# LanceZPF/loongx

Measured on AMD Instinct MI355X. Metric: edited images/s @512x512, 28-step Flux denoise, higher is better.
Workload: dtype bf16

## Files before the change

### loongx_amd/csrc/gemm.hip

```cpp
#include "gemm8.h"


static double round_us(int bm, int K) { return bm == 256 ? 15.0 + 1.81 * (K / 64) : 10.5 + 1.06 * (K / 64); }

struct GemmEnv { int bm, g4, sk, g4_fault; };
static int env_int(const char* name, int dflt) {
  const char* s = getenv(name);
  return s ? atoi(s) : dflt;
}
static GemmEnv read_gemm_env() { return GemmEnv{env_int("LX_GEMM_BM", 0), env_int("LX_GEMM4", 1), env_int("LX_GEMM4_SK", 1), env_int("LX_GEMM4_FAULT", 0)}; }
static GemmEnv g_gemm_env = read_gemm_env();
static const GemmEnv& gemm_env() { return g_gemm_env; }
extern "C" void lx_gemm_reload_env(void) { g_gemm_env = read_gemm_env(); }

namespace {
constexpr size_t SK_FLAGS_OFF = (size_t)256 * SK_SLOT_FLOATS * sizeof(float);
constexpr size_t SK_WS_BYTES = SK_FLAGS_OFF + (256 + 64) * sizeof(int);
static_assert(SK_WS_BYTES % 256 == 0, "workspace size keeps the 256-byte alignment contract");
constexpr int SK_MIN_KT_ALL = 96;
constexpr int SK_MAX_ROUNDS = 16;

int device_cus() {
  static int n = -1;
  if (n < 0) {
    int dev = 0;
    hipDeviceProp_t pr;
    n = (hipGetDevice(&dev) == hipSuccess && hipGetDeviceProperties(&pr, dev) == hipSuccess) ? pr.multiProcessorCount : 0;
  }
  return n;
}
}

static long tiles_of(const lx_gemm_desc& p, int bm) { return (long)((p.M + bm - 1) / bm) * ((p.N + BN - 1) / BN); }

static lx_gemm_desc sub_rows(const lx_gemm_desc& p, int r0, int rows) {
  lx_gemm_desc q = p;
  q.A = (const uint16_t*)p.A + (size_t)r0 * p.lda;
  const int epi = p.epilogue & 0xff;
  q.C = epi == LX_EPI_STORE_BF16 ? (void*)((uint16_t*)p.C + (size_t)r0 * p.ldc) : (void*)((float*)p.C + (size_t)r0 * p.ldc);
  if (p.lora_t) q.lora_t = p.lora_t + (size_t)r0 * p.lora_ldt;
  if (p.qkv_k) q.qkv_k = (uint16_t*)p.qkv_k + (size_t)r0 * p.qkv_k_ld;
  if (p.qkv_q8) {
    q.qkv_q8 = (uint8_t*)p.qkv_q8 + (size_t)r0 * p.qkv_ld8;
// ... 1 lines not shown
  }
  q.M = rows;
  return q;
}

static int launch_plan(const GemmArgs& a, int bm, hipStream_t s, int variant = LX_GV_BF16) {
  if (a.n == 0) return LX_OK;
  if (variant == LX_GV_SPLIT) lx_gemm8_launch_split(bm, a, s);
  else if (variant == LX_GV_F16) lx_gemm8_launch_f16(bm, a, s);
  else if (variant == LX_GV_FP8) lx_gemm8_launch_fp8(bm, a, s);
  else lx_gemm8_launch_bf16(bm, a, s);
  LX_LAUNCH_CHECK("lx_gemm_bf16");
  return LX_OK;
}

void lx_gemm8_launch_bf16(int bm, const GemmArgs& a, hipStream_t s) {
  const int t = a.tile_start[a.n];
  if (bm == 256) hipLaunchKernelGGL((lx_gemm_kernel<256, false>), dim3(t), dim3(NTHREADS), 0, s, a);
  else hipLaunchKernelGGL((lx_gemm_kernel<128, false>), dim3(t), dim3(NTHREADS), 0, s, a);
}
void lx_gemm8_mixed_launch_bf16(const GemmArgs& big, const GemmArgs& tail, int n_big_pad, hipStream_t s) {
  hipLaunchKernelGGL(lx_gemm_mixed_kernel<false>, dim3(n_big_pad + tail.tile_start[tail.n]), dim3(NTHREADS), 0, s, big, tail, n_big_pad);
}

static void plan_add(GemmArgs& a, const lx_gemm_desc& p, int m_base, int bm) {
  a.p[a.n] = p;
  a.m_base[a.n] = m_base;
  a.tile_start[a.n + 1] = a.tile_start[a.n] + (int)tiles_of(p, bm);
  ++a.n;
  for (int i = a.n + 1; i <= MAX_SUB; ++i) a.tile_start[i] = a.tile_start[a.n];
}

static thread_local int lx_gemm_last = LX_GEMM_PLAN_NONE;
extern "C" int lx_gemm_last_plan(void) { return lx_gemm_last; }
static int planned(int rc, int plan) {
  if (rc == LX_OK) lx_gemm_last = plan;
  return rc;
}

extern "C" size_t lx_gemm_workspace_bytes(void) { return SK_WS_BYTES; }

extern "C" int lx_gemm_workspace_status(void* workspace, void* stream) {
  LX_CHECK_ARG(workspace, "lx_gemm_workspace_status: NULL workspace");
  int* err = (int*)((char*)workspace + SK_FLAGS_OFF) + 256;
  int v = 0;
  hipStream_t s = (hipStream_t)stream;
  if (hipMemcpyAsync(&v, err, sizeof(int), hipMemcpyDeviceToHost, s) != hipSuccess || hipStreamSynchronize(s) != hipSuccess) {
    lx_set_error("lx_gemm_workspace_status: reading the error word failed: %s", hipGetErrorString(hipGetLastError()));
    return LX_ERR_LAUNCH;
  }
  if (v == 0) return LX_OK;
  (void)hipMemsetAsync((char*)workspace + SK_FLAGS_OFF, 0, (256 + 64) * sizeof(int), s);
  (void)hipStreamSynchronize(s);
  lx_set_error("lx_gemm_bf16_ws: a split-K pair workgroup timed out waiting for its partner (CUs held by other work?); the results "
               "of that launch are invalid. Re-run with the workspace omitted (lx_gemm_bf16) or LX_GEMM4_SK=0");
  return LX_ERR_LAUNCH;
}

extern "C" int lx_gemm_bf16(const lx_gemm_desc* problems, int n, void* stream) { return lx_gemm_bf16_ws(problems, n, nullptr, 0, stream); }

extern "C" int lx_gemm_bf16_ws(const lx_gemm_desc* problems, int n, void* workspace, size_t ws_bytes, void* stream) {
  LX_CHECK_ARG(problems && n >= 1 && n <= LX_GEMM_MAX_GROUP, "lx_gemm_bf16: n=%d out of range [1,%d]", n, LX_GEMM_MAX_GROUP);
  long t256 = 0, t128 = 0;
  int kmax = 0;
  bool split = false, fp8 = false, f16 = false, qkv = false;
  for (int i = 0; i < n; ++i) fp8 = fp8 || (problems[i].epilogue & LX_OPERANDS_FP8) != 0;
  for (int i = 0; i < n; ++i) f16 = f16 || (problems[i].epilogue & LX_OPERANDS_F16) != 0;
  for (int i = 0; i < n; ++i) {
    const lx_gemm_desc& p = problems[i];
// ... 91 lines not shown
    bool split_all = can_split && full == 0 && kt_all >= SK_MIN_KT_ALL;
    const int tail_div = !qkv && kt_all >= 96 ? 2 : 3;
    bool split_tail = can_split && full > 0 && tail * tail_div <= NCU;
    int np = 2;
    if (!split && env.sk != 2 && kt_all >= 24 && tail * 3 <= 256 && tail * 3 <= NCU && (split_all || split_tail) && (kt_all >= 96 || tail * 6 <= NCU)) np = 3;
    if (split) {
      const double r4 = 8.9 + 1.31 * kt_all;
      const bool sk_tail = can_split && tail > 0;
      const double c4 = (double)(full / NCU) * r4 + (tail == 0 ? 0.0 : sk_tail ? 8.9 + 1.31 * (kt_all - kt_all / 2) + 6.0 : r4);
      const double c8a = (double)((t256 + NCU - 1) / NCU) * (5.8 + 1.55 * kt_all), c8b = (double)((t128 + NCU - 1) / NCU) * (10.5 + 1.06 * kt_all);
      fills = env.g4 == 2 || c4 < (c8a < c8b ? c8a : c8b);
      split_all = fills && sk_tail && full == 0;
      split_tail = fills && sk_tail && full > 0;
      if (!fills) split_all = split_tail = false;
    }
    if (ok && (fills || split_all || split_tail)) {
      GemmArgs all;
      all.n = 0;
      all.tile_start[0] = 0;
      for (int i = 1; i <= MAX_SUB; ++i) all.tile_start[i] = 0;
      for (int i = 0; i < n; ++i) plan_add(all, problems[i], 0, 256);
      float* slots = nullptr;
      int *flags = nullptr, *err = nullptr;
      unsigned grid = (unsigned)t256;
      int sk_full = (int)t256, sk_parts = 1;
      if (split_all || split_tail) {
        slots = (float*)workspace;
        flags = (int*)((char*)workspace + SK_FLAGS_OFF);
        err = flags + 256;
        grid = (unsigned)(full + np * tail);
        sk_full = (int)full;
        sk_parts = env.g4_fault ? 3 : 2;
      }
      if (split) lx_gemm4_launch_split(all, grid, sk_full, sk_parts, slots, flags, err, s);
      else if (f16) lx_gemm4_launch_f16(all, grid, sk_full, sk_parts, slots, flags, err, s, np);
      else lx_gemm4_launch_bf16(all, grid, sk_full, sk_parts, slots, flags, err, s, np);
      LX_LAUNCH_CHECK("lx_gemm_bf16");
      return planned(LX_OK, !(split_all || split_tail) ? LX_GEMM_PLAN_G4 : np == 3 ? LX_GEMM_PLAN_G4_SPLIT3 : LX_GEMM_PLAN_G4_SPLIT2);
    }
  }
  if (split) {
    const double ca = (double)((t256 + NCU - 1) / NCU) * round_us(256, kmax), cb = (double)((t128 + NCU - 1) / NCU) * round_us(128, kmax);
    const int bm = forced ? forced : (cb < ca ? 128 : 256);
    GemmArgs all;
    all.n = 0;
    all.tile_start[0] = 0;
    for (int i = 1; i <= MAX_SUB; ++i) all.tile_start[i] = 0;
    for (int i = 0; i < n; ++i) plan_add(all, problems[i], 0, bm);
    return planned(launch_plan(all, bm, s, LX_GV_SPLIT), bm == 256 ? LX_GEMM_PLAN_8WAVE_256 : LX_GEMM_PLAN_8WAVE_128);
  }
  if (workspace) LX_CHECK_ARG(ws_bytes >= SK_WS_BYTES && ((uintptr_t)workspace & 255) == 0, "lx_gemm_bf16_ws: workspace needs %zu bytes (lx_gemm_workspace_bytes()), 256-byte aligned", SK_WS_BYTES);
  const int variant = f16 ? LX_GV_F16 : LX_GV_BF16;
  const double c_a = (double)((t256 + NCU - 1) / NCU) * round_us(256, kmax);
  const double c_b = (double)((t128 + NCU - 1) / NCU) * round_us(128, kmax);
  GemmArgs big, tail;
  big.n = tail.n = 0;
  big.tile_start[0] = tail.tile_start[0] = 0;
  for (int i = 1; i <= MAX_SUB; ++i) big.tile_start[i] = tail.tile_start[i] = 0;
  double c_c = 1e30;
  const long full = (t256 / NCU) * NCU;
  if (forced == 0 && full > 0 && t256 > full) {
    long remain = t256;
    int keep_rows[LX_GEMM_MAX_GROUP];
    for (int i = 0; i < n; ++i) keep_rows[i] = problems[i].M;
    for (int i = n - 1; i >= 0 && remain > full; --i) {
      const int tn = (problems[i].N + BN - 1) / BN;
      while (remain > full && keep_rows[i] > 0) {
        const int last_rows = keep_rows[i] % 256 ? keep_rows[i] % 256 : 256;
        keep_rows[i] -= last_rows;
        remain -= tn;
      }
// ... 34 lines not shown
```

### loongx_amd/csrc/gemm4.h

```cpp
#pragma once
#include "gemm_common.h"

namespace {

constexpr int G4_STAGE = 256 * BK * 2 + BN * BK * 2;
constexpr int G4_LDS = 2 * G4_STAGE;
constexpr int G4_PLD = 132;
constexpr int G4_PATCHES = 4 * 2 * 16 * G4_PLD * 4;
constexpr int G4_SLOT = 8 * 1024;
constexpr int G4_SMEM = G4_PATCHES + 4 * 2 * G4_SLOT > G4_LDS ? G4_PATCHES + 4 * 2 * G4_SLOT : G4_LDS;
static_assert(G4_LDS <= G4_SMEM && G4_SMEM <= 160 * 1024 && G4_PATCHES % 1024 == 0 && G4_PATCHES + 4 * 2 * G4_SLOT <= G4_SMEM,
              "LDS budget / epilogue patches / row ring");

#ifdef LX_G4_PROBE
__device__ unsigned long long lx_g4_probe_buf[8192 * 8];
#define G4_STAMP(k) if (threadIdx.x == 0 && blockIdx.x < 8192) { asm volatile("s_waitcnt lgkmcnt(0)" ::: "memory"); lx_g4_probe_buf[blockIdx.x * 8 + (k)] = __builtin_amdgcn_s_memtime(); }
#else
#define G4_STAMP(k)
#endif


template <bool SPLIT, bool F16 = false, int NP = 2>
__global__ __launch_bounds__(G4_THREADS) void lx_gemm4_kernel(const GemmArgs args, const int sk_full, const int sk_parts, float* __restrict__ sk_slots,
                                                              int* __restrict__ sk_flags, int* __restrict__ sk_err) {
#if defined(__HIP_DEVICE_COMPILE__)
  __shared__ __attribute__((aligned(1024))) char smem[G4_SMEM];
  constexpr int BM = 256, A_BYTES = BM * BK * 2;
  const int pid = blockIdx.x;
  G4_STAMP(0)
  const int total = args.tile_start[MAX_SUB];
  int lid, part = 0;
  if (pid < sk_full) {
    const int q = sk_full >> 3, r = sk_full & 7;
    const int xcd = pid & 7, inx = pid >> 3;
    lid = (xcd < r ? xcd * (q + 1) : r * (q + 1) + (xcd - r) * q) + inx;
  } else {
    const int r = pid - sk_full;
    lid = sk_full + r / NP;
    part = r % NP;
  }
  (void)total;
  const bool split_tile = pid >= sk_full && sk_parts >= 2;
  const int g = tile_group(args, lid);
  lx_gemm_desc P = args.p[g];
  int tm, tn;
  tile_coords<BM>(P, lid - args.tile_start[g], tm, tn);
  const int tid = threadIdx.x, lane = tid & 63;
  const int wave = __builtin_amdgcn_readfirstlane(tid >> 6);
  const int wm = wave >> 1, wn = wave & 1, l15 = lane & 15, lq = lane >> 4;
  int m0 = tm * BM, n0 = tn * BN;
  int M = P.M, N = P.N;
  const int K = P.K;
  const bool w_tiled = (P.epilogue & LX_W_TILED) != 0;
  const int nk1 = K / BK;
  const int nkt = SPLIT ? nk1 * max(P.k_segs, 1) : nk1;
// ... 188 lines not shown
    __syncthreads();
    __builtin_amdgcn_fence(__ATOMIC_RELEASE, "workgroup");
    if (tid == 0) {
      const int me = pid - sk_full, other = NP == 2 ? (me ^ 1) : (me - part + (part + 1) % NP), other2 = me - part + (part + 2) % NP;
      bool ok = __hip_atomic_load(sk_err, __ATOMIC_RELAXED, __HIP_MEMORY_SCOPE_AGENT) == 0;
      if (ok) {
        if (!(sk_parts == 3 && part == 1))
          __hip_atomic_store(sk_flags + me, NP - 1, __ATOMIC_RELAXED, __HIP_MEMORY_SCOPE_AGENT);
        int spins = 0;
        while (__hip_atomic_load(sk_flags + other, __ATOMIC_RELAXED, __HIP_MEMORY_SCOPE_AGENT) == 0) {
          __builtin_amdgcn_s_sleep(1);
          if (++spins > (1 << 20)) { ok = false; break; }
        }
        if constexpr (NP == 3) {
          while (ok && __hip_atomic_load(sk_flags + other2, __ATOMIC_RELAXED, __HIP_MEMORY_SCOPE_AGENT) == 0) {
            __builtin_amdgcn_s_sleep(1);
            if (++spins > (1 << 20)) { ok = false; break; }
          }
        }
        if (ok) {
          if constexpr (NP == 2) __hip_atomic_store(sk_flags + other, 0, __ATOMIC_RELAXED, __HIP_MEMORY_SCOPE_AGENT);
          else {
            __hip_atomic_fetch_add(sk_flags + other, -1, __ATOMIC_RELAXED, __HIP_MEMORY_SCOPE_AGENT);
            __hip_atomic_fetch_add(sk_flags + other2, -1, __ATOMIC_RELAXED, __HIP_MEMORY_SCOPE_AGENT);
          }
        } else __hip_atomic_store(sk_err, 1, __ATOMIC_RELAXED, __HIP_MEMORY_SCOPE_AGENT);
      }
    }
    __syncthreads();
    G4_STAMP(6)
    __builtin_amdgcn_fence(__ATOMIC_ACQUIRE, "workgroup");
  };

  const int epi = P.epilogue & 0xff;
  const bool do_gelu = (P.epilogue & LX_EPI_GELU) != 0;
  const int mw0 = m0 + wm * 128, nw0 = n0 + wn * 128;
  float* patch = (float*)smem + wave * (2 * 16 * G4_PLD);
  const bool bf16_out = epi == LX_EPI_STORE_BF16;
  const int c8 = (lane & 15) * 8, c4 = (lane & 31) * 4;
  const int ncol = nw0 + (bf16_out ? c8 : c4);
  const bool col_ok = ncol < N;
  f32x4 bias0 = {0.f, 0.f, 0.f, 0.f}, bias1 = {0.f, 0.f, 0.f, 0.f};
  if (P.bias && col_ok) {
    bias0 = *(const f32x4*)(P.bias + ncol);
    if (bf16_out) bias1 = *(const f32x4*)(P.bias + ncol + 4);
  }
  asm volatile("s_waitcnt vmcnt(0)" : "+v"(bias0), "+v"(bias1)::"memory");
  const bool gelu0 = do_gelu && ncol >= P.gelu_col_start;
  const int m_base = args.m_base[g];
  static_assert(!(F16 && SPLIT), "fp16 operands exclude the split-bf16 mode");
  float f16_mx = 0.f;
  const bool qkv_tile = (P.epilogue & LX_EPI_QKV) != 0 && n0 < 3 * P.qkv_d;
  const int qkind = qkv_tile ? n0 / P.qkv_d : -1;
  f32x4 nw0v = {1.f, 1.f, 1.f, 1.f}, nw1v = {1.f, 1.f, 1.f, 1.f};
  if (qkv_tile && qkind != 1) {
    const float* nwp = (qkind == 2 ? P.qkv_norm_q : P.qkv_norm_k) + c8;
    nw0v = *(const f32x4*)nwp; nw1v = *(const f32x4*)(nwp + 4);
    asm volatile("s_waitcnt vmcnt(0)" : "+v"(nw0v), "+v"(nw1v)::"memory");
  }
#ifdef LX_G4_RESID_GLOBAL
  constexpr bool RING_RES = false;
#else
  constexpr bool RING_RES = true;
#endif
#ifdef LX_G4_ROPE_GLOBAL
  constexpr bool RING_ROPE = false;
#else
  constexpr bool RING_ROPE = true;
#endif
  char* const ring = smem + G4_PATCHES + wave * (2 * G4_SLOT);
  const bool ring_res = RING_RES && epi == LX_EPI_RESID_F32 && !qkv_tile;
  const bool ring_rope = RING_ROPE && qkv_tile && qkind != 1;
  const int ring_lane = ring_rope ? ((lane >> 4) * 128 + c8) * 4 : min(ncol, max(N - 4, 0)) * 4;
  const int ring_mlast = M - 1 - mw0;
  auto ring_issue = [&](int b, int s) {
    const lx_rsrc_t rs_row = lx_make_rsrc(ring_rope ? (const void*)P.qkv_rope : (const void*)((const float*)P.C + (size_t)min(mw0, M - 1) * P.ldc));
    if (ring_rope) {
      const int gm = m_base + mw0 + b * 16, p0 = gm - (gm / P.rows_per_batch) * P.rows_per_batch;
#pragma unroll
      for (int p_ = 0; p_ < 8; ++p_)
        lx_buf_to_lds(rs_row, (lptr_t)(ring + s * G4_SLOT + p_ * 1024), (uint32_t)ring_lane, (p0 + (p_ >> 1) * 4) * 512 + (p_ & 1) * 16);
    } else {
#pragma unroll
      for (int t = 0; t < 8; ++t) {
        const int r = min(b * 16 + t * 2 + (lane >> 5), ring_mlast);
        lx_buf_to_lds(rs_row, (lptr_t)(ring + s * G4_SLOT + t * 1024), (uint32_t)(r * P.ldc * 4 + ring_lane), 0);
      }
    }
  };
  auto ring_wait = [&](auto ko_, bool nxt, bool stores, auto st_) {
    constexpr int ko = decltype(ko_)::value, ST = decltype(st_)::value, S = ST * (ko < 2 ? ko : 2);
    if (stores) {
      if (nxt) asm volatile("s_waitcnt vmcnt(%0)" ::"n"(S + 8) : "memory");
      else asm volatile("s_waitcnt vmcnt(%0)" ::"n"(S) : "memory");
    } else {
      if (nxt) asm volatile("s_waitcnt vmcnt(8)" ::: "memory");
      else asm volatile("s_waitcnt vmcnt(0)" ::: "memory");
    }
  };
  const bool gate_tile = RING_RES && epi == LX_EPI_RESID_F32 && !qkv_tile && P.gate != nullptr &&
                         (m_base + m0) / P.rows_per_batch == (m_base + m0 + BM - 1) / P.rows_per_batch;
  f32x4 gate_t = {0.f, 0.f, 0.f, 0.f};
  if (gate_tile && col_ok) gate_t = *(const f32x4*)(P.gate + (size_t)((m_base + m0) / P.rows_per_batch) * P.gate_ld + ncol);
  asm volatile("s_waitcnt vmcnt(0)" : "+v"(gate_t)::"memory");
  auto put = [&](auto ic_) {
    constexpr int i = decltype(ic_)::value;
    float* pt = patch + (i & 1) * (16 * G4_PLD);
    asm volatile("" : "+a"(acc[i][0]), "+a"(acc[i][1]), "+a"(acc[i][2]), "+a"(acc[i][3]), "+a"(acc[i][4]), "+a"(acc[i][5]), "+a"(acc[i][6]), "+a"(acc[i][7]));
#pragma unroll
    for (int j = 0; j < 8; ++j) *(f32x4*)(pt + l15 * G4_PLD + j * 16 + 4 * lq) = acc[i][j];
  };
  auto park = [&](auto ic_, auto nx_) {
    constexpr int i = decltype(ic_)::value, nx = decltype(nx_)::value;
    const float* pt = patch + (i & 1) * (16 * G4_PLD);
    __builtin_amdgcn_wave_barrier();
    if constexpr (nx >= 0) { if (mw0 + nx * 16 < M) put(std::integral_constant<int, nx>{}); }
    __builtin_amdgcn_sched_barrier(0);
    if (mw0 + i * 16 >= M) return;
    const lx_rsrc_t rs_slot = lx_make_rsrc(my_slot);
#pragma unroll
    for (int t = 0; t < 8; ++t) {
      const int row = t * 2 + (lane >> 5);
      const f32x4 v = *(const f32x4*)(pt + row * G4_PLD + c4);
      __builtin_amdgcn_raw_buffer_store_b128(u32x4{__float_as_uint(v[0]), __float_as_uint(v[1]), __float_as_uint(v[2]), __float_as_uint(v[3])}, rs_slot,
                                             (int)(((size_t)(wm * 128 + i * 16 + row) * 256 + wn * 128 + c4) * 4), 0, PAIR_AUX_SC1);
    }
  };
  auto block = [&](auto ic_, auto nx_, auto ko_, auto n2_) {
    constexpr int i = decltype(ic_)::value, nx = decltype(nx_)::value, ko = decltype(ko_)::value, n2 = decltype(n2_)::value;
    const int mb = mw0 + i * 16;
    if (mb >= M) return;
    const float* pt = patch + (i & 1) * (16 * G4_PLD);
    const char* const slot = ring + (ko & 1) * G4_SLOT + lane * 16;
    const bool ring_nxt = nx >= 0 && mw0 + nx * 16 < M;
    f32x4 res[8], gat[8];
    if (epi == LX_EPI_RESID_F32 && !qkv_tile) {
      const int rpb = P.rows_per_batch;
#pragma unroll
      for (int t = 0; t < 8; ++t) {
        const int m = mb + t * 2 + (lane >> 5);
        if (m < M && col_ok) {
          if (!RING_RES) {
            res[t] = *(const f32x4*)((const float*)P.C + (size_t)m * P.ldc + ncol);
            if (P.gate) gat[t] = *(const f32x4*)(P.gate + (size_t)((m_base + m) / rpb) * P.gate_ld + ncol);
          }
        }
      }
    }
    __builtin_amdgcn_wave_barrier();
    if constexpr (nx >= 0) { if (mw0 + nx * 16 < M) put(std::integral_constant<int, nx>{}); }
    __builtin_amdgcn_sched_barrier(0);
    if (partner) {
      f32x4 pa[4][2], pb[4][2];
#pragma unroll
      for (int t = 0; t < 4; ++t) {
        const size_t po = (size_t)(lm0 + i * 16 + t * 4 + (lane >> 4)) * 256 + ln0 + c8;
        pa[t][0] = pld4(po, partner); pa[t][1] = pld4(po + 4, partner);
        if constexpr (NP == 3) { pb[t][0] = pld4(po, partner2); pb[t][1] = pld4(po + 4, partner2); }
      }
      float* pw = patch + (i & 1) * (16 * G4_PLD);
#pragma unroll
      for (int t = 0; t < 4; ++t) {
        float* q_ = pw + (t * 4 + (lane >> 4)) * G4_PLD + c8;
        f32x4 v0 = *(const f32x4*)q_, v1 = *(const f32x4*)(q_ + 4);
#pragma unroll
        for (int c_ = 0; c_ < 4; ++c_) { v0[c_] += pa[t][0][c_]; v1[c_] += pa[t][1][c_]; }
        if constexpr (NP == 3) {
#pragma unroll
          for (int c_ = 0; c_ < 4; ++c_) { v0[c_] += pb[t][0][c_]; v1[c_] += pb[t][1][c_]; }
        }
        *(f32x4*)q_ = v0; *(f32x4*)(q_ + 4) = v1;
      }
      __builtin_amdgcn_wave_barrier();
    }
    if (qkv_tile) {
      const int D = P.qkv_d, L = P.rows_per_batch, H = D >> 7;
      const int gm = m_base + mb, b = gm / L, p0 = gm - b * L;
      const int h = (nw0 - qkind * D) >> 7;
      if (qkind == 1) {
        const int gk = lane & 1;
        float e[4][8];
#pragma unroll
        for (int t = 0; t < 4; ++t)
#pragma unroll
          for (int k = 0; k < 8; ++k) {
            const int rk = lx_vt_interleave(gk * 8 + k), dk = t * 32 + (lane >> 1);
            e[t][k] = pt[rk * G4_PLD + dk];
          }
#pragma unroll
        for (int t = 0; t < 4; ++t) {
          const int d = t * 32 + (lane >> 1);
          const float bd = P.bias ? P.bias[nw0 + d] : 0.f;
          u32x4 o = {pack_bf16x2(e[t][0] + bd, e[t][1] + bd), pack_bf16x2(e[t][2] + bd, e[t][3] + bd), pack_bf16x2(e[t][4] + bd, e[t][5] + bd),
                     pack_bf16x2(e[t][6] + bd, e[t][7] + bd)};
          *(u32x4*)((uint16_t*)P.qkv_vt + ((size_t)(b * H + h) * 128 + d) * P.qkv_vt_ld + P.qkv_vt_pos0 + p0 + gk * 8) = o;
        }
      } else {
        uint16_t* const out = (qkind == 0 && P.qkv_k) ? (uint16_t*)P.qkv_k : (uint16_t*)P.C;
        const int out_ld = (qkind == 0 && P.qkv_k) ? P.qkv_k_ld : P.ldc;
        f32x4 cs[4][2], pv[4][2];
        if constexpr (RING_ROPE) {
          ring_wait(ko_, ring_nxt, true, std::integral_constant<int, 4>{});
#pragma unroll
          for (int t = 0; t < 4; ++t) { cs[t][0] = *(const f32x4*)(slot + (t * 2) * 1024); cs[t][1] = *(const f32x4*)(slot + (t * 2 + 1) * 1024); }
        } else {
#pragma unroll
          for (int t = 0; t < 4; ++t) {
            const float* rp = P.qkv_rope + (size_t)(p0 + t * 4 + (lane >> 4)) * 128 + c8;
// ... 15 lines not shown
#pragma unroll
        for (int t = 0; t < 4; ++t) {
          f32x4 v0 = pv[t][0], v1 = pv[t][1];
          float ss = 0.f;
#pragma unroll
          for (int c_ = 0; c_ < 4; ++c_) { v0[c_] += bias0[c_]; v1[c_] += bias1[c_]; ss = __builtin_fmaf(v0[c_], v0[c_], ss); ss = __builtin_fmaf(v1[c_], v1[c_], ss); }
#ifdef LX_G4_ROW16_SHFL
          ss += __shfl_xor(ss, 1, 64); ss += __shfl_xor(ss, 2, 64); ss += __shfl_xor(ss, 4, 64); ss += __shfl_xor(ss, 8, 64);
#else
          ss = row16_sum(ss);
#endif
          const float r = rsqrtf(ss * (1.0f / 128.0f) + 1e-6f);
          float x[8];
          float (&y)[8] = yy[t];
#pragma unroll
          for (int c_ = 0; c_ < 4; ++c_) { x[c_] = v0[c_] * r * nw0v[c_]; x[4 + c_] = v1[c_] * r * nw1v[c_]; }
#pragma unroll
          for (int q = 0; q < 4; ++q) {
            const float co = q < 2 ? cs[t][0][2 * q] : cs[t][1][2 * q - 4], si = q < 2 ? cs[t][0][2 * q + 1] : cs[t][1][2 * q - 3];
            y[2 * q] = x[2 * q] * co - x[2 * q + 1] * si;
            y[2 * q + 1] = x[2 * q + 1] * co + x[2 * q] * si;
          }
        }
#pragma unroll
        for (int t = 0; t < 4; ++t) {
          const int m = mb + t * 4 + (lane >> 4);
          const float (&y)[8] = yy[t];
          u32x4 o = {pack_bf16x2(y[0], y[1]), pack_bf16x2(y[2], y[3]), pack_bf16x2(y[4], y[5]), pack_bf16x2(y[6], y[7])};
          if (m < M) *(u32x4*)(out + (size_t)m * out_ld + ncol) = o;
        }
      }
      return;
    }
    if (bf16_out) {
      f32x4 pv[4][2];
#pragma unroll
      for (int t = 0; t < 4; ++t) {
        const int row = t * 4 + (lane >> 4);
        pv[t][0] = *(const f32x4*)(pt + row * G4_PLD + c8); pv[t][1] = *(const f32x4*)(pt + row * G4_PLD + c8 + 4);
      }
#pragma unroll
      for (int t = 0; t < 4; ++t) {
        const int row = t * 4 + (lane >> 4), m = mb + row;
        f32x4 v0 = pv[t][0], v1 = pv[t][1];
        if (m < M && col_ok) {
#pragma unroll
          for (int c_ = 0; c_ < 4; ++c_) { v0[c_] += bias0[c_]; v1[c_] += bias1[c_]; }
          if (gelu0) { v0 = gelu_tanh4(v0); v1 = gelu_tanh4(v1); }
          u32x4 o = {pack_op16x2<F16>(v0[0], v0[1], f16_mx), pack_op16x2<F16>(v0[2], v0[3], f16_mx), pack_op16x2<F16>(v1[0], v1[1], f16_mx),
                     pack_op16x2<F16>(v1[2], v1[3], f16_mx)};
          *(u32x4*)((uint16_t*)P.C + (size_t)m * P.ldc + ncol) = o;
          if constexpr (SPLIT) {
            if (P.epilogue & LX_EPI_SPLIT_BF16) {
              float r[8];
#pragma unroll
              for (int c_ = 0; c_ < 4; ++c_) {
                r[c_] = v0[c_] - bf16_to_f32(f32_to_bf16(v0[c_]));
                r[4 + c_] = v1[c_] - bf16_to_f32(f32_to_bf16(v1[c_]));
              }
              u32x4 ol = {pack_bf16x2(r[0], r[1]), pack_bf16x2(r[2], r[3]), pack_bf16x2(r[4], r[5]), pack_bf16x2(r[6], r[7])};
              *(u32x4*)((uint16_t*)P.C + (size_t)m * P.ldc + ncol + P.c_lo_off) = ol;
            }
          }
        }
      }
    } else {
      f32x4 pv[8];
#pragma unroll
      for (int t = 0; t < 8; ++t) pv[t] = *(const f32x4*)(pt + (t * 2 + (lane >> 5)) * G4_PLD + c4);
      if (epi == LX_EPI_RESID_F32) {
        if constexpr (RING_RES) {
          if (P.gate && !gate_tile) {
            const int rpb = P.rows_per_batch;
#pragma unroll
            for (int t = 0; t < 8; ++t) {
              const int m = mb + t * 2 + (lane >> 5);
              if (m < M && col_ok) gat[t] = *(const f32x4*)(P.gate + (size_t)((m_base + m) / rpb) * P.gate_ld + ncol);
            }
            asm volatile("s_waitcnt vmcnt(0)" ::: "memory");
#pragma unroll
            for (int t = 0; t < 8; ++t) asm volatile("" : "+v"(gat[t]));
          } else ring_wait(ko_, ring_nxt, nw0 < N, std::integral_constant<int, 8>{});
#pragma unroll
          for (int t = 0; t < 8; ++t) res[t] = *(const f32x4*)(slot + t * 1024);
          asm volatile("s_waitcnt lgkmcnt(0)" : "+v"(res[0]), "+v"(res[1]), "+v"(res[2]), "+v"(res[3]), "+v"(res[4]), "+v"(res[5]), "+v"(res[6]), "+v"(res[7])::"memory");
          if constexpr (n2 >= 0) { if (mw0 + n2 * 16 < M) ring_issue(n2, ko & 1); }
        } else {
          asm volatile("s_waitcnt vmcnt(0)" ::: "memory");
#pragma unroll
          for (int t = 0; t < 8; ++t) asm volatile("" : "+v"(res[t]), "+v"(gat[t]));
        }
      }
#pragma unroll
      for (int t = 0; t < 8; ++t) {
        const int row = t * 2 + (lane >> 5), m = mb + row;
        f32x4 v = pv[t];
        if (m < M && col_ok) {
#pragma unroll
          for (int c_ = 0; c_ < 4; ++c_) v[c_] += bias0[c_];
          if (gelu0) v = gelu_tanh4(v);
          if (epi == LX_EPI_RESID_F32) {
            f32x4 o = res[t];
            if (P.gate) {
              const f32x4 gv = gate_tile ? gate_t : gat[t];
#pragma unroll
              for (int c_ = 0; c_ < 4; ++c_) o[c_] = __builtin_fmaf(gv[c_], v[c_], o[c_]);
            } else {
#pragma unroll
              for (int c_ = 0; c_ < 4; ++c_) o[c_] += v[c_];
            }
            v = o;
          }
          *(f32x4*)((float*)P.C + (size_t)m * P.ldc + ncol) = v;
        }
      }
    }
  };
#define G4_B(I, NX, KO, N2) block(std::integral_constant<int, I>{}, std::integral_constant<int, NX>{}, std::integral_constant<int, KO>{}, std::integral_constant<int, N2>{})
#define G4_K(I, NX) park(std::integral_constant<int, I>{}, std::integral_constant<int, NX>{})
#define G4_R(B0, B1) if (ring_res || ring_rope) { if (mw0 + (B0) * 16 < M) ring_issue(B0, 0); if (mw0 + (B1) * 16 < M) ring_issue(B1, 1); }
  if (!split_tile) {
    G4_R(0, 1)
    if (mw0 < M) put(std::integral_constant<int, 0>{});
    G4_B(0, 1, 0, 2); G4_B(1, 2, 1, 3); G4_B(2, 3, 2, 4); G4_B(3, 4, 3, 5); G4_B(4, 5, 4, 6); G4_B(5, 6, 5, 7); G4_B(6, 7, 6, -1); G4_B(7, -1, 7, -1);
  } else if constexpr (NP == 2) {
    if (part == 0) {
      G4_R(0, 1)
      if (mw0 + 64 < M) put(std::integral_constant<int, 4>{});
      G4_K(4, 5); G4_K(5, 6); G4_K(6, 7); G4_K(7, 0);
      exchange();
      G4_B(0, 1, 0, 2); G4_B(1, 2, 1, 3); G4_B(2, 3, 2, -1); G4_B(3, -1, 3, -1);
    } else {
      G4_R(4, 5)
      if (mw0 < M) put(std::integral_constant<int, 0>{});
      G4_K(0, 1); G4_K(1, 2); G4_K(2, 3); G4_K(3, 4);
      exchange();
      G4_B(4, 5, 0, 6); G4_B(5, 6, 1, 7); G4_B(6, 7, 2, -1); G4_B(7, -1, 3, -1);
    }
  } else {
    if (part == 0) {
      G4_R(0, 1)
      if (mw0 + 48 < M) put(std::integral_constant<int, 3>{});
      G4_K(3, 4); G4_K(4, 5); G4_K(5, 6); G4_K(6, 7); G4_K(7, 0);
      exchange();
      G4_B(0, 1, 0, 2); G4_B(1, 2, 1, -1); G4_B(2, -1, 2, -1);
    } else if (part == 1) {
      G4_R(3, 4)
      if (mw0 < M) put(std::integral_constant<int, 0>{});
      G4_K(0, 1); G4_K(1, 2); G4_K(2, 7); G4_K(7, 6); G4_K(6, 3);
      exchange();
      G4_B(3, 4, 0, 5); G4_B(4, 5, 1, -1); G4_B(5, -1, 2, -1);
    } else {
      G4_R(6, 7)
      if (mw0 < M) put(std::integral_constant<int, 0>{});
      G4_K(0, 1); G4_K(1, 2); G4_K(2, 3); G4_K(3, 4); G4_K(4, 5); G4_K(5, 6);
      exchange();
      G4_B(6, 7, 0, -1); G4_B(7, -1, 1, -1);
    }
  }
#undef G4_B
#undef G4_K
#undef G4_R
  if constexpr (F16) { if (bf16_out && !qkv_tile) report_f16_overflow(f16_mx, P.f16_ovf); }
  asm volatile("s_waitcnt vmcnt(0)" ::: "memory");
  G4_STAMP(5)
#endif
}


}
```

### loongx_amd/csrc/gemm4.hip

```cpp
#include "gemm4.h"

void lx_gemm4_launch_bf16(const GemmArgs& a, unsigned grid, int sk_full, int sk_parts, float* slots, int* flags, int* err, hipStream_t s, int np) {
  if (np == 3) hipLaunchKernelGGL((lx_gemm4_kernel<false, false, 3>), dim3(grid), dim3(G4_THREADS), 0, s, a, sk_full, sk_parts, slots, flags, err);
  else hipLaunchKernelGGL((lx_gemm4_kernel<false, false>), dim3(grid), dim3(G4_THREADS), 0, s, a, sk_full, sk_parts, slots, flags, err);
}

#ifdef LX_G4_PROBE
extern "C" int lx_g4_probe_read(unsigned long long* host, size_t n_u64) {
  return hipMemcpyFromSymbol(host, HIP_SYMBOL(lx_g4_probe_buf), n_u64 * sizeof(unsigned long long), 0, hipMemcpyDeviceToHost) == hipSuccess ? 0 : -1;
}
#endif
```

### loongx_amd/csrc/gemm4_f16.hip

```cpp
#include "gemm4.h"

void lx_gemm4_launch_f16(const GemmArgs& a, unsigned grid, int sk_full, int sk_parts, float* slots, int* flags, int* err, hipStream_t s, int np) {
  if (np == 3) hipLaunchKernelGGL((lx_gemm4_kernel<false, true, 3>), dim3(grid), dim3(G4_THREADS), 0, s, a, sk_full, sk_parts, slots, flags, err);
  else hipLaunchKernelGGL((lx_gemm4_kernel<false, true>), dim3(grid), dim3(G4_THREADS), 0, s, a, sk_full, sk_parts, slots, flags, err);
}
```

### loongx_amd/csrc/gemm_common.h

```cpp
#pragma once
#include "common.h"
#include <type_traits>

constexpr int MAX_SUB = 2 * LX_GEMM_MAX_GROUP;

struct GemmArgs {
  lx_gemm_desc p[MAX_SUB];
  int tile_start[MAX_SUB + 1];
  int m_base[MAX_SUB];
  int n;
};
static_assert(2 * sizeof(GemmArgs) + 16 <= 4096, "lx_gemm_mixed_kernel takes two plans by value: the kernarg segment is 4 KiB");

namespace {

constexpr int BN = 256;
constexpr int BK = 64;
constexpr int NTHREADS = 512;
#ifndef LX_GROUP_M
#define LX_GROUP_M 4
#endif
constexpr int GROUP_M = LX_GROUP_M;

typedef const __attribute__((address_space(1))) void* gptr_t;
// ... 4 lines not shown
__device__ __forceinline__ int tile_group(const GemmArgs& args, const int lid) {
  int g = 0;
#pragma unroll
  for (int i = 1; i < MAX_SUB; ++i)
    if (lid >= args.tile_start[i]) g = i;
  return g;
}

template <int BM>
__device__ __forceinline__ void tile_coords(const lx_gemm_desc& P, const int local, int& tm, int& tn) {
  const int tiles_m = (P.M + BM - 1) / BM;
  const int tiles_n = (P.N + BN - 1) / BN;
  const int gs = GROUP_M * tiles_n;
  const int gi = local / gs, in_g = local - gi * gs;
  const int first_m = gi * GROUP_M;
  const int gm = min(tiles_m - first_m, GROUP_M);
  tm = first_m + in_g % gm;
  tn = in_g / gm;
}

constexpr int G4_THREADS = 256;
constexpr int SK_SLOT_FLOATS = 256 * 256;

}

enum { LX_GV_BF16 = 0, LX_GV_F16 = 1, LX_GV_SPLIT = 2, LX_GV_FP8 = 3 };

void lx_gemm8_launch_bf16(int bm, const GemmArgs& a, hipStream_t s);
void lx_gemm8_launch_f16(int bm, const GemmArgs& a, hipStream_t s);
void lx_gemm8_launch_split(int bm, const GemmArgs& a, hipStream_t s);
void lx_gemm8_launch_fp8(int bm, const GemmArgs& a, hipStream_t s);
void lx_gemm8_mixed_launch_bf16(const GemmArgs& big, const GemmArgs& tail, int n_big_pad, hipStream_t s);
void lx_gemm8_mixed_launch_f16(const GemmArgs& big, const GemmArgs& tail, int n_big_pad, hipStream_t s);
void lx_gemm4_launch_bf16(const GemmArgs& a, unsigned grid, int sk_full, int sk_parts, float* slots, int* flags, int* err, hipStream_t s, int np = 2);
void lx_gemm4_launch_f16(const GemmArgs& a, unsigned grid, int sk_full, int sk_parts, float* slots, int* flags, int* err, hipStream_t s, int np = 2);
void lx_gemm4_launch_split(const GemmArgs& a, unsigned grid, int sk_full, int sk_parts, float* slots, int* flags, int* err, hipStream_t s);
```

Measured before the change: 1.025.

## Specialize gemm4 epilogue per launch and add a 16-bit patch store path

Adds an EPI_SET template parameter to the gemm4 kernel so launches whose subproblems all share one epilogue (plain bf16 store, qkv/bf16 store, or f32 residual) compile only that branch. This drops dead code and register pressure. For the plain bf16-store set it adds a new epilogue that applies bias and GELU in registers, packs to 16-bit, and stages through a swizzled 16-bit LDS patch before writing full rows. This replaces the f32 patch round-trip. It adds more template instantiations, a host-side classification step, and new LDS layout logic that could hide bank conflicts or correctness issues.

Result: no change. 1.032, median of 6 (+0.7%).

```diff
diff --git a/loongx_amd/csrc/gemm.hip b/loongx_amd/csrc/gemm.hip
--- a/loongx_amd/csrc/gemm.hip
+++ b/loongx_amd/csrc/gemm.hip
@@ -3,12 +3,12 @@
 
 static double round_us(int bm, int K) { return bm == 256 ? 15.0 + 1.81 * (K / 64) : 10.5 + 1.06 * (K / 64); }
 
-struct GemmEnv { int bm, g4, sk, g4_fault; };
+struct GemmEnv { int bm, g4, sk, g4_fault, epi_sets; };
 static int env_int(const char* name, int dflt) {
   const char* s = getenv(name);
   return s ? atoi(s) : dflt;
 }
-static GemmEnv read_gemm_env() { return GemmEnv{env_int("LX_GEMM_BM", 0), env_int("LX_GEMM4", 1), env_int("LX_GEMM4_SK", 1), env_int("LX_GEMM4_FAULT", 0)}; }
+static GemmEnv read_gemm_env() { return GemmEnv{env_int("LX_GEMM_BM", 0), env_int("LX_GEMM4", 1), env_int("LX_GEMM4_SK", 1), env_int("LX_GEMM4_FAULT", 0), env_int("LX_GEMM4_EPI_SETS", 1)}; }
 static GemmEnv g_gemm_env = read_gemm_env();
 static const GemmEnv& gemm_env() { return g_gemm_env; }
 extern "C" void lx_gemm_reload_env(void) { g_gemm_env = read_gemm_env(); }
@@ -76,9 +76,11 @@
 }
 
 static thread_local int lx_gemm_last = LX_GEMM_PLAN_NONE;
+static thread_local int lx_gemm_last_set = -1;
 extern "C" int lx_gemm_last_plan(void) { return lx_gemm_last; }
-static int planned(int rc, int plan) {
-  if (rc == LX_OK) lx_gemm_last = plan;
+extern "C" int lx_gemm_last_epi_set(void) { return lx_gemm_last_set; }
+static int planned(int rc, int plan, int epi_set = -1) {
+  if (rc == LX_OK) { lx_gemm_last = plan; lx_gemm_last_set = epi_set; }
   return rc;
 }
 
@@ -236,11 +238,22 @@
         sk_full = (int)full;
         sk_parts = env.g4_fault ? 3 : 2;
       }
+      int epi_set = G4_EPI_ALL;
+      if (!split && env.epi_sets) {
+        bool all16 = true, all_res = true;
+        for (int i = 0; i < n; ++i) {
+          const int e = problems[i].epilogue & 0xff;
+          all16 = all16 && e == LX_EPI_STORE_BF16;
+          all_res = all_res && e == LX_EPI_RESID_F32 && !(problems[i].epilogue & (LX_EPI_GELU | LX_EPI_QKV));
+        }
+        if (all16) epi_set = (qkv || split_all || split_tail) ? G4_EPI_QKV_STORE16 : G4_EPI_STORE16;
+        else if (all_res) epi_set = G4_EPI_RESID;
+      }
       if (split) lx_gemm4_launch_split(all, grid, sk_full, sk_parts, slots, flags, err, s);
-      else if (f16) lx_gemm4_launch_f16(all, grid, sk_full, sk_parts, slots, flags, err, s, np);
-      else lx_gemm4_launch_bf16(all, grid, sk_full, sk_parts, slots, flags, err, s, np);
+      else if (f16) lx_gemm4_launch_f16(all, grid, sk_full, sk_parts, slots, flags, err, s, np, epi_set);
+      else lx_gemm4_launch_bf16(all, grid, sk_full, sk_parts, slots, flags, err, s, np, epi_set);
       LX_LAUNCH_CHECK("lx_gemm_bf16");
-      return planned(LX_OK, !(split_all || split_tail) ? LX_GEMM_PLAN_G4 : np == 3 ? LX_GEMM_PLAN_G4_SPLIT3 : LX_GEMM_PLAN_G4_SPLIT2);
+      return planned(LX_OK, !(split_all || split_tail) ? LX_GEMM_PLAN_G4 : np == 3 ? LX_GEMM_PLAN_G4_SPLIT3 : LX_GEMM_PLAN_G4_SPLIT2, epi_set);
     }
   }
   if (split) {
diff --git a/loongx_amd/csrc/gemm4.h b/loongx_amd/csrc/gemm4.h
--- a/loongx_amd/csrc/gemm4.h
+++ b/loongx_amd/csrc/gemm4.h
@@ -20,7 +20,7 @@
 #endif
 
 
-template <bool SPLIT, bool F16 = false, int NP = 2>
+template <bool SPLIT, bool F16 = false, int NP = 2, int EPI_SET = G4_EPI_ALL>
 __global__ __launch_bounds__(G4_THREADS) void lx_gemm4_kernel(const GemmArgs args, const int sk_full, const int sk_parts, float* __restrict__ sk_slots,
                                                               int* __restrict__ sk_flags, int* __restrict__ sk_err) {
 #if defined(__HIP_DEVICE_COMPILE__)
@@ -275,8 +275,14 @@
     __builtin_amdgcn_fence(__ATOMIC_ACQUIRE, "workgroup");
   };
 
-  const int epi = P.epilogue & 0xff;
-  const bool do_gelu = (P.epilogue & LX_EPI_GELU) != 0;
+  constexpr bool E_ALL = EPI_SET == G4_EPI_ALL;
+  constexpr bool E_RND = EPI_SET == G4_EPI_STORE16;
+  constexpr bool E_QKV = E_ALL || EPI_SET == G4_EPI_QKV_STORE16;
+  constexpr bool E_ST16 = E_ALL || EPI_SET == G4_EPI_QKV_STORE16;
+  constexpr bool E_F32 = E_ALL || EPI_SET == G4_EPI_RESID;
+  static_assert(E_ALL || !SPLIT, "the split-bf16 mode runs the all-in-one body");
+  const int epi = E_ALL ? (P.epilogue & 0xff) : EPI_SET == G4_EPI_RESID ? (int)LX_EPI_RESID_F32 : (int)LX_EPI_STORE_BF16;
+  const bool do_gelu = EPI_SET != G4_EPI_RESID && (P.epilogue & LX_EPI_GELU) != 0;
   const int mw0 = m0 + wm * 128, nw0 = n0 + wn * 128;
   float* patch = (float*)smem + wave * (2 * 16 * G4_PLD);
   const bool bf16_out = epi == LX_EPI_STORE_BF16;
@@ -284,16 +290,18 @@
   const int ncol = nw0 + (bf16_out ? c8 : c4);
   const bool col_ok = ncol < N;
   f32x4 bias0 = {0.f, 0.f, 0.f, 0.f}, bias1 = {0.f, 0.f, 0.f, 0.f};
-  if (P.bias && col_ok) {
-    bias0 = *(const f32x4*)(P.bias + ncol);
-    if (bf16_out) bias1 = *(const f32x4*)(P.bias + ncol + 4);
-  }
-  asm volatile("s_waitcnt vmcnt(0)" : "+v"(bias0), "+v"(bias1)::"memory");
+  if constexpr (!E_RND) {
+    if (P.bias && col_ok) {
+      bias0 = *(const f32x4*)(P.bias + ncol);
+      if (bf16_out) bias1 = *(const f32x4*)(P.bias + ncol + 4);
+    }
+    asm volatile("s_waitcnt vmcnt(0)" : "+v"(bias0), "+v"(bias1)::"memory");
+  }
   const bool gelu0 = do_gelu && ncol >= P.gelu_col_start;
   const int m_base = args.m_base[g];
   static_assert(!(F16 && SPLIT), "fp16 operands exclude the split-bf16 mode");
   float f16_mx = 0.f;
-  const bool qkv_tile = (P.epilogue & LX_EPI_QKV) != 0 && n0 < 3 * P.qkv_d;
+  const bool qkv_tile = E_QKV && (P.epilogue & LX_EPI_QKV) != 0 && n0 < 3 * P.qkv_d;
   const int qkind = qkv_tile ? n0 / P.qkv_d : -1;
   f32x4 nw0v = {1.f, 1.f, 1.f, 1.f}, nw1v = {1.f, 1.f, 1.f, 1.f};
   if (qkv_tile && qkind != 1) {
@@ -312,13 +320,14 @@
   constexpr bool RING_ROPE = true;
 #endif
   char* const ring = smem + G4_PATCHES + wave * (2 * G4_SLOT);
-  const bool ring_res = RING_RES && epi == LX_EPI_RESID_F32 && !qkv_tile;
-  const bool ring_rope = RING_ROPE && qkv_tile && qkind != 1;
+  const bool ring_res = E_F32 && RING_RES && epi == LX_EPI_RESID_F32 && !qkv_tile;
+  const bool ring_rope = E_QKV && RING_ROPE && qkv_tile && qkind != 1;
   const int ring_lane = ring_rope ? ((lane >> 4) * 128 + c8) * 4 : min(ncol, max(N - 4, 0)) * 4;
   const int ring_mlast = M - 1 - mw0;
   auto ring_issue = [&](int b, int s) {
-    const lx_rsrc_t rs_row = lx_make_rsrc(ring_rope ? (const void*)P.qkv_rope : (const void*)((const float*)P.C + (size_t)min(mw0, M - 1) * P.ldc));
-    if (ring_rope) {
+    const bool rope = !E_F32 || (E_QKV && ring_rope);
+    const lx_rsrc_t rs_row = lx_make_rsrc(rope ? (const void*)P.qkv_rope : (const void*)((const float*)P.C + (size_t)min(mw0, M - 1) * P.ldc));
+    if (rope) {
       const int gm = m_base + mw0 + b * 16, p0 = gm - (gm / P.rows_per_batch) * P.rows_per_batch;
 #pragma unroll
       for (int p_ = 0; p_ < 8; ++p_)
@@ -341,17 +350,28 @@
       else asm volatile("s_waitcnt vmcnt(0)" ::: "memory");
     }
   };
-  const bool gate_tile = RING_RES && epi == LX_EPI_RESID_F32 && !qkv_tile && P.gate != nullptr &&
+  const bool gate_tile = E_F32 && RING_RES && epi == LX_EPI_RESID_F32 && !qkv_tile && P.gate != nullptr &&
                          (m_base + m0) / P.rows_per_batch == (m_base + m0 + BM - 1) / P.rows_per_batch;
   f32x4 gate_t = {0.f, 0.f, 0.f, 0.f};
-  if (gate_tile && col_ok) gate_t = *(const f32x4*)(P.gate + (size_t)((m_base + m0) / P.rows_per_batch) * P.gate_ld + ncol);
-  asm volatile("s_waitcnt vmcnt(0)" : "+v"(gate_t)::"memory");
+  if constexpr (E_F32) {
+    if (gate_tile && col_ok) gate_t = *(const f32x4*)(P.gate + (size_t)((m_base + m0) / P.rows_per_batch) * P.gate_ld + ncol);
+    asm volatile("s_waitcnt vmcnt(0)" : "+v"(gate_t)::"memory");
+  }
+#ifdef LX_G4_ELIM_PATCH
+  f32x4 elim_hold[2][8];
+#endif
   auto put = [&](auto ic_) {
     constexpr int i = decltype(ic_)::value;
     float* pt = patch + (i & 1) * (16 * G4_PLD);
     asm volatile("" : "+a"(acc[i][0]), "+a"(acc[i][1]), "+a"(acc[i][2]), "+a"(acc[i][3]), "+a"(acc[i][4]), "+a"(acc[i][5]), "+a"(acc[i][6]), "+a"(acc[i][7]));
+#ifdef LX_G4_ELIM_PATCH
+#pragma unroll
+    for (int j = 0; j < 8; ++j) elim_hold[i & 1][j] = acc[i][j];
+    (void)pt;
+#else
 #pragma unroll
     for (int j = 0; j < 8; ++j) *(f32x4*)(pt + l15 * G4_PLD + j * 16 + 4 * lq) = acc[i][j];
+#endif
   };
   auto park = [&](auto ic_, auto nx_) {
     constexpr int i = decltype(ic_)::value, nx = decltype(nx_)::value;
@@ -416,7 +436,7 @@
       }
       __builtin_amdgcn_wave_barrier();
     }
-    if (qkv_tile) {
+    if constexpr (E_QKV) if (qkv_tile) {
       const int D = P.qkv_d, L = P.rows_per_batch, H = D >> 7;
       const int gm = m_base + mb, b = gm / L, p0 = gm - b * L;
       const int h = (nw0 - qkind * D) >> 7;
@@ -498,12 +518,17 @@
       }
       return;
     }
-    if (bf16_out) {
+    if constexpr (E_ST16) if (bf16_out) {
       f32x4 pv[4][2];
 #pragma unroll
       for (int t = 0; t < 4; ++t) {
         const int row = t * 4 + (lane >> 4);
+#ifdef LX_G4_ELIM_PATCH
+        pv[t][0] = elim_hold[i & 1][2 * t]; pv[t][1] = elim_hold[i & 1][2 * t + 1];
+        (void)row;
+#else
         pv[t][0] = *(const f32x4*)(pt + row * G4_PLD + c8); pv[t][1] = *(const f32x4*)(pt + row * G4_PLD + c8 + 4);
+#endif
       }
 #pragma unroll
       for (int t = 0; t < 4; ++t) {
@@ -512,10 +537,16 @@
         if (m < M && col_ok) {
 #pragma unroll
           for (int c_ = 0; c_ < 4; ++c_) { v0[c_] += bias0[c_]; v1[c_] += bias1[c_]; }
+#ifndef LX_G4_ELIM_GELU
           if (gelu0) { v0 = gelu_tanh4(v0); v1 = gelu_tanh4(v1); }
+#endif
           u32x4 o = {pack_op16x2<F16>(v0[0], v0[1], f16_mx), pack_op16x2<F16>(v0[2], v0[3], f16_mx), pack_op16x2<F16>(v1[0], v1[1], f16_mx),
                      pack_op16x2<F16>(v1[2], v1[3], f16_mx)};
+#ifdef LX_G4_ELIM_STORE
+          asm volatile("" ::"v"(o));
+#else
           *(u32x4*)((uint16_t*)P.C + (size_t)m * P.ldc + ncol) = o;
+#endif
           if constexpr (SPLIT) {
             if (P.epilogue & LX_EPI_SPLIT_BF16) {
               float r[8];
@@ -530,7 +561,9 @@
           }
         }
       }
-    } else {
+      return;
+    }
+    if constexpr (E_F32) {
       f32x4 pv[8];
 #pragma unroll
       for (int t = 0; t < 8; ++t) pv[t] = *(const f32x4*)(pt + (t * 2 + (lane >> 5)) * G4_PLD + c4);
@@ -582,10 +615,82 @@
       }
     }
   };
+  constexpr int G4_PLD16 = 272;
+  static_assert(4 * 4 * 16 * G4_PLD16 <= G4_SMEM, "four 16-bit patches per wave");
+  char* const patch16 = smem + wave * (4 * 16 * G4_PLD16);
+  f32x4 bj[8];
+  int jg = 8;
+  bool cj_ok[8];
+  if constexpr (E_RND) {
+#pragma unroll
+    for (int j = 0; j < 8; ++j) {
+      const int cj = nw0 + j * 16 + 4 * lq;
+      cj_ok[j] = cj < N;
+      bj[j] = f32x4{0.f, 0.f, 0.f, 0.f};
+      if (P.bias && cj_ok[j]) bj[j] = *(const f32x4*)(P.bias + cj);
+    }
+#pragma unroll
+    for (int j = 7; j >= 0; --j)
+      if (do_gelu && ((nw0 + j * 16 + 4 * lq) & ~7) >= P.gelu_col_start) jg = j;
+    asm volatile("s_waitcnt vmcnt(0)" : "+v"(bj[0]), "+v"(bj[1]), "+v"(bj[2]), "+v"(bj[3]), "+v"(bj[4]), "+v"(bj[5]), "+v"(bj[6]), "+v"(bj[7])::"memory");
+  }
+  const bool gelu_wave = E_RND && do_gelu && nw0 + 120 >= P.gelu_col_start;
+  auto put16 = [&](auto ic_) {
+    constexpr int i = decltype(ic_)::value;
+    char* const pt = patch16 + (i & 3) * (16 * G4_PLD16) + l15 * G4_PLD16 + ((lq * 8) ^ (l15 & 8));
+    asm volatile("" : "+a"(acc[i][0]), "+a"(acc[i][1]), "+a"(acc[i][2]), "+a"(acc[i][3]), "+a"(acc[i][4]), "+a"(acc[i][5]), "+a"(acc[i][6]), "+a"(acc[i][7]));
+    f32x4 v[8];
+#pragma unroll
+    for (int j = 0; j < 8; ++j)
+#pragma unroll
+      for (int c_ = 0; c_ < 4; ++c_) v[j][c_] = acc[i][j][c_] + bj[j][c_];
+    if (gelu_wave) {
+#pragma unroll
+      for (int j = 0; j < 8; ++j) {
+        const f32x4 gv = gelu_tanh4(v[j]);
+        if (j >= jg) v[j] = gv;
+      }
+    }
+    const bool row_ok = mw0 + i * 16 + l15 < M;
+#pragma unroll
+    for (int j = 0; j < 8; ++j) {
+      float mx = f16_mx;
+      const u32x2 o = {pack_op16x2<F16>(v[j][0], v[j][1], mx), pack_op16x2<F16>(v[j][2], v[j][3], mx)};
+      if constexpr (F16) { if (row_ok && cj_ok[j]) f16_mx = mx; }
+      *(u32x2*)(pt + j * 32) = o;
+    }
+    asm volatile("" ::: "memory");
+  };
+  auto block16 = [&](auto ic_, auto nx_) {
+    constexpr int i = decltype(ic_)::value, nx = decltype(nx_)::value;
+    const int mb = mw0 + i * 16;
+    if (mb >= M) return;
+    const char* const pt = patch16 + (i & 3) * (16 * G4_PLD16) + (lane >> 4) * G4_PLD16 + (lane & 15) * 16;
+    __builtin_amdgcn_wave_barrier();
+    u32x4 o[4];
+#pragma unroll
+    for (int t = 0; t < 4; ++t) {
+      const u32x4 x = *(const u32x4*)(pt + t * 4 * G4_PLD16);
+      o[t] = t >= 2 ? u32x4{x[2], x[3], x[0], x[1]} : x;
+    }
+    __builtin_amdgcn_sched_barrier(0);
+    if constexpr (nx >= 0) { if (mw0 + nx * 16 < M) put16(std::integral_constant<int, nx>{}); }
+    __builtin_amdgcn_sched_barrier(0);
+#pragma unroll
+    for (int t = 0; t < 4; ++t) {
+      const int m = mb + t * 4 + (lane >> 4);
+      if (m < M && col_ok) *(u32x4*)((uint16_t*)P.C + (size_t)m * P.ldc + ncol) = o[t];
+    }
+  };
 #define G4_B(I, NX, KO, N2) block(std::integral_constant<int, I>{}, std::integral_constant<int, NX>{}, std::integral_constant<int, KO>{}, std::integral_constant<int, N2>{})
 #define G4_K(I, NX) park(std::integral_constant<int, I>{}, std::integral_constant<int, NX>{})
 #define G4_R(B0, B1) if (ring_res || ring_rope) { if (mw0 + (B0) * 16 < M) ring_issue(B0, 0); if (mw0 + (B1) * 16 < M) ring_issue(B1, 1); }
-  if (!split_tile) {
+#define G4_B16(I, NX) block16(std::integral_constant<int, I>{}, std::integral_constant<int, NX>{})
+  if constexpr (E_RND) {
+    if (mw0 < M) put16(std::integral_constant<int, 0>{});
+    if (mw0 + 16 < M) put16(std::integral_constant<int, 1>{});
+    G4_B16(0, 2); G4_B16(1, 3); G4_B16(2, 4); G4_B16(3, 5); G4_B16(4, 6); G4_B16(5, 7); G4_B16(6, -1); G4_B16(7, -1);
+  } else if (!split_tile) {
     G4_R(0, 1)
     if (mw0 < M) put(std::integral_constant<int, 0>{});
     G4_B(0, 1, 0, 2); G4_B(1, 2, 1, 3); G4_B(2, 3, 2, 4); G4_B(3, 4, 3, 5); G4_B(4, 5, 4, 6); G4_B(5, 6, 5, 7); G4_B(6, 7, 6, -1); G4_B(7, -1, 7, -1);
@@ -624,6 +729,7 @@
       G4_B(6, 7, 0, -1); G4_B(7, -1, 1, -1);
     }
   }
+#undef G4_B16
 #undef G4_B
 #undef G4_K
 #undef G4_R
@@ -633,5 +739,16 @@
 #endif
 }
 
-
+template <bool F16>
+void g4_launch_set(const GemmArgs& a, unsigned grid, int sk_full, int sk_parts, float* slots, int* flags, int* err, hipStream_t s, int np, int epi_set) {
+#define G4_GO(NP_, SET_) hipLaunchKernelGGL((lx_gemm4_kernel<false, F16, NP_, SET_>), dim3(grid), dim3(G4_THREADS), 0, s, a, sk_full, sk_parts, slots, flags, err)
+  if (epi_set == G4_EPI_STORE16) G4_GO(2, G4_EPI_STORE16);
+  else if (epi_set == G4_EPI_QKV_STORE16) { if (np == 3) G4_GO(3, G4_EPI_QKV_STORE16); else G4_GO(2, G4_EPI_QKV_STORE16); }
+  else if (epi_set == G4_EPI_RESID) { if (np == 3) G4_GO(3, G4_EPI_RESID); else G4_GO(2, G4_EPI_RESID); }
+  else if (np == 3) G4_GO(3, G4_EPI_ALL);
+  else G4_GO(2, G4_EPI_ALL);
+#undef G4_GO
 }
+
+
+}
diff --git a/loongx_amd/csrc/gemm4.hip b/loongx_amd/csrc/gemm4.hip
--- a/loongx_amd/csrc/gemm4.hip
+++ b/loongx_amd/csrc/gemm4.hip
@@ -1,8 +1,7 @@
 #include "gemm4.h"
 
-void lx_gemm4_launch_bf16(const GemmArgs& a, unsigned grid, int sk_full, int sk_parts, float* slots, int* flags, int* err, hipStream_t s, int np) {
-  if (np == 3) hipLaunchKernelGGL((lx_gemm4_kernel<false, false, 3>), dim3(grid), dim3(G4_THREADS), 0, s, a, sk_full, sk_parts, slots, flags, err);
-  else hipLaunchKernelGGL((lx_gemm4_kernel<false, false>), dim3(grid), dim3(G4_THREADS), 0, s, a, sk_full, sk_parts, slots, flags, err);
+void lx_gemm4_launch_bf16(const GemmArgs& a, unsigned grid, int sk_full, int sk_parts, float* slots, int* flags, int* err, hipStream_t s, int np, int epi_set) {
+  g4_launch_set<false>(a, grid, sk_full, sk_parts, slots, flags, err, s, np, epi_set);
 }
 
 #ifdef LX_G4_PROBE
diff --git a/loongx_amd/csrc/gemm4_f16.hip b/loongx_amd/csrc/gemm4_f16.hip
--- a/loongx_amd/csrc/gemm4_f16.hip
+++ b/loongx_amd/csrc/gemm4_f16.hip
@@ -1,6 +1,5 @@
 #include "gemm4.h"
 
-void lx_gemm4_launch_f16(const GemmArgs& a, unsigned grid, int sk_full, int sk_parts, float* slots, int* flags, int* err, hipStream_t s, int np) {
-  if (np == 3) hipLaunchKernelGGL((lx_gemm4_kernel<false, true, 3>), dim3(grid), dim3(G4_THREADS), 0, s, a, sk_full, sk_parts, slots, flags, err);
-  else hipLaunchKernelGGL((lx_gemm4_kernel<false, true>), dim3(grid), dim3(G4_THREADS), 0, s, a, sk_full, sk_parts, slots, flags, err);
+void lx_gemm4_launch_f16(const GemmArgs& a, unsigned grid, int sk_full, int sk_parts, float* slots, int* flags, int* err, hipStream_t s, int np, int epi_set) {
+  g4_launch_set<true>(a, grid, sk_full, sk_parts, slots, flags, err, s, np, epi_set);
 }
diff --git a/loongx_amd/csrc/gemm_common.h b/loongx_amd/csrc/gemm_common.h
--- a/loongx_amd/csrc/gemm_common.h
+++ b/loongx_amd/csrc/gemm_common.h
@@ -60,6 +60,9 @@
 void lx_gemm8_launch_fp8(int bm, const GemmArgs& a, hipStream_t s);
 void lx_gemm8_mixed_launch_bf16(const GemmArgs& big, const GemmArgs& tail, int n_big_pad, hipStream_t s);
 void lx_gemm8_mixed_launch_f16(const GemmArgs& big, const GemmArgs& tail, int n_big_pad, hipStream_t s);
-void lx_gemm4_launch_bf16(const GemmArgs& a, unsigned grid, int sk_full, int sk_parts, float* slots, int* flags, int* err, hipStream_t s, int np = 2);
-void lx_gemm4_launch_f16(const GemmArgs& a, unsigned grid, int sk_full, int sk_parts, float* slots, int* flags, int* err, hipStream_t s, int np = 2);
+enum { G4_EPI_ALL = 0, G4_EPI_STORE16 = 1, G4_EPI_QKV_STORE16 = 2, G4_EPI_RESID = 3 };
+void lx_gemm4_launch_bf16(const GemmArgs& a, unsigned grid, int sk_full, int sk_parts, float* slots, int* flags, int* err, hipStream_t s, int np = 2,
+                          int epi_set = G4_EPI_ALL);
+void lx_gemm4_launch_f16(const GemmArgs& a, unsigned grid, int sk_full, int sk_parts, float* slots, int* flags, int* err, hipStream_t s, int np = 2,
+                         int epi_set = G4_EPI_ALL);
 void lx_gemm4_launch_split(const GemmArgs& a, unsigned grid, int sk_full, int sk_parts, float* slots, int* flags, int* err, hipStream_t s);
```
